# Duy1230/Map-Reduced-Approach-for-Vietnamese-Long-Document-Summarization

Measured on AMD Instinct MI355X. Metric: map-phase chunks/sec (2k-tok chunk, 256-tok summary) at 1/2/4/8 MI355X, higher is better.
Workload: dtype f16

## Files before the change

include/mapsum.h:

```cpp
#ifndef MAPSUM_H
#define MAPSUM_H

#include <stddef.h>
#include <stdint.h>

#ifdef __cplusplus
extern "C" {
#endif

#define MS_ABI_VERSION 3

#define MS_OK 0
#define MS_EIO -5
#define MS_ENOMEM -12
#define MS_EBUSY -16
#define MS_EINVAL -22
#define MS_ENOSPC -28

#define MS_FINISH_EOS 1
#define MS_FINISH_LENGTH 2
#define MS_FINISH_ERROR 3

#define MS_FLAG_IGNORE_EOS 1u

// ... 44 lines not shown
  int64_t finished;
  double prefill_ms, decode_ms;
  double kernel_ms[8];
  int64_t kernel_launches[8];
  int64_t decode_kv_tokens;
  int64_t graphs_built;
  int64_t persist_fallbacks;
  int64_t persist_steps;
} ms_stats;

typedef struct ms_engine ms_engine;

int ms_create(const ms_config* cfg, ms_engine** out);
int ms_destroy(ms_engine* e);
const char* ms_last_error(const ms_engine* e);

int ms_load_weight(ms_engine* e, int32_t tensor, int32_t layer, const uint16_t* host_f16,
                   int64_t n_elems);
int ms_init_synthetic(ms_engine* e, uint64_t seed, float std, float norm_jitter);

#define MS_GGML_Q4_K 12
#define MS_GGML_Q6_K 14
int ms_load_weight_q(ms_engine* e, int32_t tensor, int32_t layer, int32_t ggml_type,
                     const void* host_blocks, int64_t n_bytes);
int ms_init_synthetic_q(ms_engine* e, uint64_t seed, float scale, float norm_jitter);

int ms_weight_regions(const ms_engine* e, void** ptrs, int64_t* bytes, int32_t cap);
int ms_quant_manifest(const ms_engine* e, int32_t* triples, int32_t cap);
int ms_declare_weight_q(ms_engine* e, int32_t tensor, int32_t layer, int32_t ggml_type);

int ms_submit(ms_engine* e, const int32_t* ids, int32_t n, int32_t num_predict,
              uint32_t flags, uint64_t tag);
#define MS_SAMPLE_MAX_TOPK 256
#define MS_SAMPLE_MAX_WINDOW 256
typedef struct ms_sampling {
  float temperature;
  int32_t top_k;
  float top_p;
  float min_p;
  float repeat_penalty;
  int32_t repeat_last_n;
  uint64_t seed;
} ms_sampling;
int ms_submit_sampled(ms_engine* e, const int32_t* ids, int32_t n, int32_t num_predict,
                      uint32_t flags, uint64_t tag, const ms_sampling* sp);
int ms_set_eos_ids(ms_engine* e, const int32_t* ids, int32_t n);
int ms_step(ms_engine* e);
int ms_poll(ms_engine* e, ms_result* out, int32_t cap);
int ms_pending(const ms_engine* e);
int ms_get_stats(const ms_engine* e, ms_stats* out);
int ms_reset_stats(ms_engine* e);
int ms_set_profiling(ms_engine* e, uint32_t class_mask);
int ms_trace_push(const char* name);
int ms_trace_pop(void);
int ms_synchronize(ms_engine* e);
int ms_set_persist(ms_engine* e, int32_t on);
#define MS_DBG_KPOOL 0
#define MS_DBG_VPOOL 1
#define MS_DBG_DECODE_LOGITS 2
#define MS_DBG_DECODE_X 3
#define MS_DBG_PREFILL_LOGITS 4
int ms_debug_read(ms_engine* e, int32_t which, int64_t offset, void* host, int64_t bytes);
int ms_debug_pk_stamps(uint64_t* out, int32_t n);
int ms_debug_a2_stamps(uint64_t* out, int32_t n);

int ms_forward(ms_engine* e, const int32_t* ids, int32_t n, int32_t n_layers_run,
               float* hidden_out, float* logits_out);
int ms_forward_packed(ms_engine* e, const int32_t* ids, const int32_t* lens, int32_t n_seqs,
                      int32_t n_layers_run, float* hidden_out, float* logits_out);
int ms_submit_forced(ms_engine* e, const int32_t* ids, int32_t n, const int32_t* forced,
                     int32_t n_forced, int32_t num_predict, uint32_t flags, uint64_t tag);

#define MS_EPI_STORE_F16 0
#define MS_EPI_ADD_F32 1
#define MS_EPI_SWIGLU 2
#define MS_EPI_STORE_F32 3
#define MS_EPI_ARGMAX 5
int ms_op_gemm(const void* A, const void* W, void* out, int32_t M, int32_t N, int32_t K,
               int32_t ldo, int32_t epilogue, void* stream);
int ms_op_gemm_resid(const void* A, const void* W, float* x, void* xg_out, const void* gamma, float* ssq_out,
                     int32_t M, int32_t N, int32_t K, void* stream);
int ms_gemm_resid_tiles(int32_t M, int32_t N);
int ms_set_gemm_variant(int32_t variant);
int ms_set_qgemv_gs(int32_t on);
int ms_set_attn_tuning(int32_t combine_grp, int32_t order);
int ms_set_dgemm_kh(int32_t kh);
int ms_set_dgemm_wn(int32_t wn);
int64_t ms_op_gemv_workspace(int32_t M, int32_t N, int32_t K);
int ms_op_gemv(const void* X, const void* W, void* out, int32_t M, int32_t N, int32_t K,
               int32_t ldo, int32_t epilogue, void* workspace, void* stream);
int ms_op_gemv_tuned(const void* X, const void* W, void* out, int32_t M, int32_t N, int32_t K,
                     int32_t ldo, int32_t epilogue, void* workspace, int32_t waves, void* stream);
int ms_op_gemv_strided(const void* X, const void* W, void* out, int32_t M, int32_t N, int32_t K,
                       int32_t ldk, int32_t ldo, int32_t epilogue, void* stream);
int ms_op_gemv_resid(const void* X, const void* W, float* x, void* xg_out, const void* gamma,
                     float* ssq_out, int32_t M, int32_t N, int32_t K, int32_t rt, void* stream);
int ms_op_set_row_scale(const float* ssq, int32_t tiles, int32_t hidden, float eps);
int ms_op_dgemm(const void* X, const void* W, void* out, int32_t M, int32_t N, int32_t K, int32_t S,
                int32_t ldo, int32_t epilogue, void* stream);
int ms_op_gemv_split(const void* X, const void* W, float* slabs, int32_t M, int32_t N, int32_t K,
                     int32_t S, int32_t waves, void* stream);
int ms_op_residual_rmsnorm(float* x, const float* slabs, int32_t S, const void* w, void* y, float* ssq,
                           int32_t rows, int32_t hidden, void* stream);
int ms_op_dequant(int32_t ggml_type, const void* blocks, int64_t n_blocks, float* out, void* stream);
int ms_op_quant_rows(int32_t ggml_type, const void* blocks, int32_t rows, int32_t K, void* f16_out,
                     void* packed_out, void* stream);
int ms_op_qgemv(const void* X, int32_t ggml_type, const void* packed_rows, void* out, int32_t M,
                int32_t N, int32_t K, int32_t ldo, int32_t epilogue, void* stream);
int ms_op_qgemv_split(const void* X, int32_t ggml_type, const void* packed_rows, float* slabs,
                      int32_t M, int32_t N, int32_t K, int32_t S, void* stream);
int ms_op_qdgemm(const void* X, int32_t ggml_type, const void* packed_rows, void* out, int32_t M,
                 int32_t N, int32_t K, int32_t S, int32_t ldo, int32_t epilogue, void* stream);
int ms_op_rmsnorm(const void* x, const void* w, void* y, float* ssq, int32_t rows, int32_t hidden,
                  const int32_t* row_idx, void* stream);
int ms_op_argmax(const void* logits, int32_t rows, int32_t n, int32_t* ids, void* stream);
int ms_op_argmax_partials(const void* partials, int32_t rows, int32_t tiles, int32_t* ids, void* stream);
int ms_op_sample(const float* logits, int32_t rows, int32_t n, int64_t ldl, const ms_sampling* params,
                 const int32_t* win, const int32_t* win_len, const int32_t* steps, int32_t* ids,
                 int32_t* cand_ids, float* cand_p, int32_t* cand_n, void* stream);

#ifdef __cplusplus
}
#endif
#endif
```

map-reduced-approach-for-vietnamese-long-document-summarization_amd/csrc/engine.cpp:

```cpp
#include <hip/hip_runtime.h>

#include <algorithm>
#include <cmath>
#include <cstddef>
#include <cstdio>
#include <cstdlib>
#include <cstring>
#include <deque>
#include <array>
#include <functional>
#include <map>
#include <tuple>
#include <memory>
#include <stdexcept>
#include <string>
#include <vector>

#if MS_HAVE_ROCTX
#include <rocprofiler-sdk-roctx/roctx.h>
#else
static inline int roctxRangePushA(const char*) { return 0; }
static inline int roctxRangePop() { return 0; }
#endif

// ... 1803 lines not shown
    } catch (...) {
      if (lg) (void)hipFree(lg);
      for (Seq& s : seqs) release(E, s);
      throw;
    }
    if (lg) (void)hipFree(lg);
    for (Seq& s : seqs) release(E, s);
    E.ev_pending.clear();
    E.ev_used = 0;
    return MS_OK;
  });
}

int ms_forward(ms_engine* e, const int32_t* ids, int32_t n, int32_t n_layers_run, float* hidden_out,
               float* logits_out) {
  return ms_forward_packed(e, ids, &n, 1, n_layers_run, hidden_out, logits_out);
}

static int op_guard(const std::function<void()>& fn) {
  try {
    fn();
    hipError_t err = hipGetLastError();
    if (err != hipSuccess) {
      g_last_error = std::string("kernel launch failed: ") + hipGetErrorString(err);
      return MS_EIO;
    }
    return MS_OK;
  } catch (const MsError& x) {
    g_last_error = x.what();
    return x.code;
  }
}

static thread_local RowScale g_op_rs{};

int ms_op_set_row_scale(const float* ssq, int32_t tiles, int32_t hidden, float eps) {
  if (ssq && (tiles < 1 || hidden < 1)) return MS_EINVAL;
  g_op_rs = ssq ? make_row_scale(ssq, tiles, hidden, eps) : RowScale{};
  return MS_OK;
}

static int op_rs_tiles() { return g_op_rs.ssq ? g_op_rs.tiles : 0; }

static const GemvArgs* op_gemv_args(GemvArgs& ga) {
  ga = GemvArgs{};
  ga.rs = g_op_rs;
  return g_op_rs.ssq ? &ga : nullptr;
}

int ms_op_gemm(const void* A, const void* W, void* out, int32_t M, int32_t N, int32_t K, int32_t ldo,
               int32_t epi, void* stream) {
  return op_guard([&] {
    REQUIRE(A && W && out && M >= 1 && N >= 16 && K >= 64 && K % 64 == 0, MS_EINVAL, "bad gemm shape");
    REQUIRE(((epi >= 0 && epi <= 3) || epi == MS_EPI_ARGMAX) && (epi != MS_EPI_SWIGLU || N % 32 == 0), MS_EINVAL,
            "bad epilogue");
    REQUIRE(epi != MS_EPI_ADD_F32 || (N % 4 == 0 && ldo % 4 == 0), MS_EINVAL,
            "residual gemm: N and ldo multiples of 4 (16-B x rows)");
    REQUIRE(epi != MS_EPI_ARGMAX || (N % 16 == 0 && ldo >= N / 16), MS_EINVAL, "gemm argmax: N % 16, ldo >= N / 16");
    REQUIRE(((uintptr_t)out & ((epi == MS_EPI_ADD_F32 || epi == MS_EPI_STORE_F32) ? 15 : 7)) == 0, MS_EINVAL,
            "gemm: out must be 16-B (fp32) / 8-B (fp16) aligned");
    REQUIRE(!g_op_rs.ssq || gemm_rs_tiles_ok(M, N, g_op_rs.tiles), MS_EINVAL,
            "gemm row scale: at most 24 tiles of statistics (kGemmRsTiles, both GEMM tiles)");
    launch_gemm((const f16_t*)A, (const f16_t*)W, out, M, N, K, ldo, epi == MS_EPI_ARGMAX ? MS_GEMV_EPI_ARGMAX : epi,
                (hipStream_t)stream, &g_op_rs);
  });
}

int ms_op_gemm_resid(const void* A, const void* W, float* x, void* xg_out, const void* gamma, float* ssq_out,
                     int32_t M, int32_t N, int32_t K, void* stream) {
  return op_guard([&] {
    REQUIRE(A && W && x && xg_out && gamma && ssq_out && M >= 1 && N >= 16 && K >= 64 && K % 64 == 0, MS_EINVAL,
            "bad gemm_resid operands (K % 64 == 0)");
    REQUIRE(gemm_resid_tiles(M, N) <= kGemmRsTiles, MS_EINVAL, "gemm_resid: N over 24 column tiles");
    REQUIRE(N % 4 == 0 && ((uintptr_t)x & 15) == 0 && ((uintptr_t)xg_out & 7) == 0, MS_EINVAL,
            "gemm_resid: N a multiple of 4, x 16-B and xg 8-B aligned (vector rows)");
    GemmResid gr{(const f16_t*)gamma, (f16_t*)xg_out, ssq_out};
    launch_gemm((const f16_t*)A, (const f16_t*)W, x, M, N, K, N, MS_EPI_ADD_F32, (hipStream_t)stream, nullptr, &gr);
  });
}

int ms_gemm_resid_tiles(int32_t M, int32_t N) { return gemm_resid_tiles(M, N); }

int ms_set_gemm_variant(int32_t v) {
  if (v < 0 || v > 4) return MS_EINVAL;
  set_gemm_variant(v);
  return MS_OK;
}

int ms_set_attn_tuning(int32_t combine_grp, int32_t order) {
  if (combine_grp < 0 || combine_grp > 1 || (order != 0 && order != 3)) return MS_EINVAL;
  set_attn_tuning(combine_grp, order);
  return MS_OK;
}

int ms_set_dgemm_kh(int32_t kh) {
  if (kh != 1 && kh != 2) return MS_EINVAL;
  set_dgemm_kh(kh);
  return MS_OK;
}

int ms_set_dgemm_wn(int32_t wn) {
  if (wn != 4 && wn != 8) return MS_EINVAL;
  set_dgemm_wn(wn);
  return MS_OK;
}

int ms_set_qgemv_gs(int32_t on) {
  if (on < 0 || on > 1) return MS_EINVAL;
  set_qgemv_gs(on != 0);
  return MS_OK;
}

int64_t ms_op_gemv_workspace(int32_t M, int32_t N, int32_t K) {
  if (M < 1 || M > 64 || N < 16 || K < 64 || K % 64) return MS_EINVAL;
  return (int64_t)gemv_workspace_bytes(M, N, K);
}

int ms_op_gemv(const void* X, const void* W, void* out, int32_t M, int32_t N, int32_t K, int32_t ldo,
               int32_t epi, void* ws, void* stream) {
  return ms_op_gemv_tuned(X, W, out, M, N, K, ldo, epi, ws, 0, stream);
}

int ms_op_gemv_tuned(const void* X, const void* W, void* out, int32_t M, int32_t N, int32_t K,
                     int32_t ldo, int32_t epi, void* ws, int32_t waves, void* stream) {
  return op_guard([&] {
    REQUIRE(X && W && out && ws && N >= 16 && N % 16 == 0, MS_EINVAL, "bad gemv operands");
    REQUIRE(((epi >= 0 && epi <= 3) || epi == MS_EPI_ARGMAX) && (epi != MS_EPI_SWIGLU || N % 32 == 0),
            MS_EINVAL, "bad epilogue");
    REQUIRE(gemv_supported(M, N, K, epi, op_rs_tiles()), MS_EINVAL,
            "gemv shape unsupported (M<=64, K%64==0, K/64 split into <=16 waves of <=8 steps; "
            "row-scale statistics within kRsStage and LDS)");
    GemvArgs ga;
    launch_gemv_ex((const f16_t*)X, (const f16_t*)W, out, M, N, K, ldo, epi, op_gemv_args(ga), waves,
                   (hipStream_t)stream);
  });
}

int ms_op_gemv_strided(const void* X, const void* W, void* out, int32_t M, int32_t N, int32_t K,
                       int32_t ldk, int32_t ldo, int32_t epi, void* stream) {
  return op_guard([&] {
    REQUIRE(X && W && out && N >= 16 && N % 16 == 0 && ldk >= K && ldk % 8 == 0, MS_EINVAL,
            "bad strided gemv operands");
    REQUIRE(epi >= 0 && epi <= 3 && epi != MS_EPI_SWIGLU, MS_EINVAL, "bad epilogue");
    REQUIRE(gemv_supported(M, N, K, epi), MS_EINVAL, "gemv shape unsupported");
    launch_gemv_strided((const f16_t*)X, (const f16_t*)W, out, M, N, K, ldk, ldo, epi, (hipStream_t)stream);
  });
}

int ms_op_gemv_resid(const void* X, const void* W, float* x, void* xg_out, const void* gamma,
                     float* ssq_out, int32_t M, int32_t N, int32_t K, int32_t rt, void* stream) {
  return op_guard([&] {
    REQUIRE(X && W && x && xg_out && gamma && ssq_out && rt >= 1 && rt <= 16 && N % rt == 0, MS_EINVAL,
            "bad gemv_resid operands");
    REQUIRE(gemv_supported(M, N, K, MS_GEMV_EPI_RESID_SSQ), MS_EINVAL, "gemv_resid shape unsupported");
    GemvArgs ga{};
    ga.rt = rt;
    ga.ssq_out = ssq_out;
    ga.gamma = (const f16_t*)gamma;
    ga.xg_out = (f16_t*)xg_out;
    launch_gemv_ex((const f16_t*)X, (const f16_t*)W, x, M, N, K, N, MS_GEMV_EPI_RESID_SSQ, &ga, 0,
                   (hipStream_t)stream);
  });
}

int ms_op_dgemm(const void* X, const void* W, void* out, int32_t M, int32_t N, int32_t K, int32_t S,
                int32_t ldo, int32_t epi, void* stream) {
  return op_guard([&] {
    REQUIRE(X && W && out, MS_EINVAL, "bad dgemm operands");
// ... 164 lines not shown
```

map-reduced-approach-for-vietnamese-long-document-summarization_amd/csrc/k_gemm.hip:

```cpp
#include "kernels.h"

namespace ms {

constexpr int GBM = 128, GBN = 128, GBK = 64;

__device__ __forceinline__ int xcd_remap(int b, int nwg) {
  const int q = nwg / 8, r = nwg % 8, x = b % 8;
  return (x < r ? x * (q + 1) : r * (q + 1) + (x - r) * q) + b / 8;
}

__device__ __forceinline__ float silu_mul(float g, float u) {
  return g * __builtin_amdgcn_rcpf(1.0f + __expf(-g)) * u;
}

template <int BM, int NW>
__device__ __forceinline__ void gemm_rs_dma(const RowScale& rs, int M, int m0, float* rinv_s, float* stage) {
  if (!rs.ssq) return;
  const int lane = threadIdx.x & 63, wave = threadIdx.x >> 6;
  if (rs.tiles == 1) {
    if (wave < BM / 64)
      __builtin_amdgcn_global_load_lds((const void*)(rs.ssq + min(m0 + wave * 64 + lane, M - 1)),
                                       (LDS_AS void*)(rinv_s + wave * 64), 4, 0, 0);
    return;
  }
// ... 578 lines not shown
      mf1(1, 4 * g + 3);
      __builtin_amdgcn_sched_barrier(0);
    }
    __builtin_amdgcn_s_setprio(0);
  }
  asm volatile("s_nop 7\n\ts_nop 7\n\ts_nop 7\n\ts_nop 7" ::: "memory");

  if constexpr (EPI == 1) {
    const bool fuse = gr.xg != nullptr;
    float* red = (float*)smem;
    if (fuse) __syncthreads();
#pragma unroll
    for (int mi = 0; mi < 8; ++mi) {
      const int row = m0 + wr * 128 + mi * 16 + fr;
      float ss[2] = {0.f, 0.f};
#pragma unroll
      for (int ni = 0; ni < 8; ++ni) {
        const int col = n0 + wc * 128 + ni * 16 + 4 * fg;
        if (row < M && col < N)
          gemm_resid_x4(gr, (float*)out, (size_t)row * ldo + col, acc[mi][ni], g8[ni], fuse, ss[ni >> 2]);
      }
      if (fuse)
#pragma unroll
        for (int h = 0; h < 2; ++h) red[((wr * 128 + mi * 16 + fr) * 2 + wc) * 8 + h * 4 + fg] = ss[h];
    }
    if (fuse) gemm_resid_ssq_t<TBM, 2>(red, M, N, m0, n0, gr);
    return;
  }
  gemm_rs_fold<TBM, kGemmRsTiles>(rs, rinv_s, rs_stage);
  {
    float rv[8];
#pragma unroll
    for (int mi = 0; mi < 8; ++mi) rv[mi] = 1.f;
    if (rs.ssq) {
#pragma unroll
      for (int mi = 0; mi < 8; ++mi) rv[mi] = rs_rinv(rinv_s[wr * 128 + mi * 16 + fr], rs);
    }
    const bool vec = (ldo & 3) == 0;
#pragma unroll
    for (int mi = 0; mi < 8; ++mi) {
      const int row = m0 + wr * 128 + mi * 16 + fr;
      if (row >= M) continue;
      if constexpr (EPI == 2) {
#pragma unroll
        for (int ni = 0; ni < 8; ni += 2) {
          const int col = n0 + wc * 128 + ni * 16;
          if (col >= N) continue;
          const int f = (col >> 5) * 16 + 4 * fg;
          float hv[4];
#pragma unroll
          for (int j = 0; j < 4; ++j) hv[j] = silu_mul(acc[mi][ni][j] * rv[mi], acc[mi][ni + 1][j] * rv[mi]);
          f16_t* o = (f16_t*)out + (size_t)row * ldo + f;
          if (vec) {
            *(uint2*)o = uint2{pack2h(hv[0], hv[1]), pack2h(hv[2], hv[3])};
          } else {
#pragma unroll
            for (int j = 0; j < 4; ++j) o[j] = f2h(hv[j]);
          }
        }
      } else {
#pragma unroll
        for (int ni = 0; ni < 8; ++ni) {
          const int col = n0 + wc * 128 + ni * 16 + 4 * fg;
          if (col >= N) continue;
          const size_t o = (size_t)row * ldo + col;
          const f32x4 v = acc[mi][ni] * rv[mi];
          if (vec && col + 3 < N) {
            if constexpr (EPI == 0) *(uint2*)((f16_t*)out + o) = uint2{pack2h(v[0], v[1]), pack2h(v[2], v[3])};
            else *(f32x4*)((float*)out + o) = v;
          } else {
#pragma unroll
            for (int j = 0; j < 4; ++j)
              if (col + j < N) {
                if constexpr (EPI == 0) ((f16_t*)out)[o + j] = f2h(v[j]);
                else ((float*)out)[o + j] = v[j];
              }
          }
        }
      }
    }
  }
}

static int g_gemm_variant = [] { const char* e = getenv("MS_GEMM_VARIANT"); return e ? atoi(e) : 4; }();

void set_gemm_variant(int v) { g_gemm_variant = v; }

static bool gemm_big(int M, int N) {
  return g_gemm_variant == 2 || g_gemm_variant == 3 ||
         ((g_gemm_variant == 0 || g_gemm_variant == 4) && M >= 1024 && N >= 1024);
}
static bool gemm_4wave(int epi) { return g_gemm_variant == 3 || (g_gemm_variant == 4 && epi != 1); }

int gemm_resid_tiles(int M, int N) {
  (void)M;
  return (N + kGemmStatCols - 1) / kGemmStatCols;
}

void launch_gemm(const f16_t* A, const f16_t* W, void* out, int M, int N, int K, int ldo, int epi,
                 hipStream_t s, const RowScale* rs_in, const GemmResid* gr_in) {
  if (M <= 0) return;
  if (epi == MS_GEMV_EPI_ARGMAX) {
    const int grid = ((M + GBM - 1) / GBM) * ((N + GBN - 1) / GBN);
    MS_LAUNCH(gemm_kernel<MS_GEMV_EPI_ARGMAX>, dim3(grid), dim3(256), 0, s, A, W, out, M, N, K, ldo, RowScale{},
              GemmResid{});
    return;
  }
  const bool big = gemm_big(M, N);
  RowScale rs{};
  if (rs_in && rs_in->ssq && epi != 1) {
    if (rs_in->tiles < 1 || rs_in->tiles > kGemmRsTiles) return;
    rs = *rs_in;
  }
  GemmResid gr{};
  if (gr_in && epi == 1) gr = *gr_in;
#define GL(KERN, EPI_, BLK) MS_LAUNCH(KERN<EPI_>, dim3(grid), dim3(BLK), 0, s, A, W, out, M, N, K, ldo, rs, gr)
  if (big && gemm_4wave(epi) && K % TBK == 0) {
    const int grid = ((M + TBM - 1) / TBM) * ((N + TBN - 1) / TBN);
    switch (epi) {
      case 0: GL(gemm4w_kernel, 0, 256); break;
      case 1: GL(gemm4w_kernel, 1, 256); break;
      case 2: GL(gemm4w_kernel, 2, 256); break;
      default: GL(gemm4w_kernel, 3, 256); break;
    }
    return;
  }
  if (big) {
    const int grid = ((M + TBM - 1) / TBM) * ((N + TBN - 1) / TBN);
    switch (epi) {
      case 0: GL(gemm256_kernel, 0, 512); break;
      case 1: GL(gemm256_kernel, 1, 512); break;
      case 2: GL(gemm256_kernel, 2, 512); break;
      default: GL(gemm256_kernel, 3, 512); break;
    }
    return;
  }
  const int grid = ((M + GBM - 1) / GBM) * ((N + GBN - 1) / GBN);
  switch (epi) {
    case 0: GL(gemm_kernel, 0, 256); break;
    case 1: GL(gemm_kernel, 1, 256); break;
    case 2: GL(gemm_kernel, 2, 256); break;
    default: GL(gemm_kernel, 3, 256); break;
  }
#undef GL
}

bool gemm_rs_tiles_ok(int M, int N, int tiles) {
  (void)M;
  (void)N;
  return tiles >= 1 && tiles <= kGemmRsTiles;
}

}
```

map-reduced-approach-for-vietnamese-long-document-summarization_amd/csrc/kernels.h:

```cpp
#pragma once
#include "common.h"

namespace ms {

struct KVView {
  f16_t* k;
  f16_t* v;
  const int32_t* block_table;
  int32_t max_pages;
  int32_t n_kv_heads;
  int32_t slot_major;
};

constexpr int kPrefillQRows = 128;
struct PrefillAttnArgs {
  const int32_t* seq_qstart;
  const int32_t* seq_qlen;
  const int32_t* seq_kvlen;
  const int32_t* seq_slot;
  const int32_t* qblk;
  int32_t n_qblk;
  const float* cos_tab;
  const float* sin_tab;
};
// ... 1 lines not shown
struct DecodeAttnArgs {
  const int32_t* seq_len;
  const int32_t* seq_slot;
  int32_t B;
  int32_t max_len;
  int32_t ppw;
};

struct RowScale {
  const float* ssq;
  int tiles, H;
  float eps;
  float inv_h;
};
inline RowScale make_row_scale(const float* ssq, int tiles, int H, float eps) {
  return RowScale{ssq, tiles, H, eps, 1.0f / (float)H};
}
constexpr float kXgScale = 0.0625f, kXgUnscale = 16.0f;
__device__ __forceinline__ float rs_rinv(float sum, const RowScale& rs) {
  return __builtin_amdgcn_rsqf(__fmaf_rn(sum, rs.inv_h, rs.eps)) * kXgUnscale;
}

void launch_embed(const int32_t* ids, int T, const f16_t* emb, int H, float* x, hipStream_t s,
                  const f16_t* gamma = nullptr, f16_t* xg = nullptr, float* ssq = nullptr);
void launch_decode_advance(int32_t* args, const int32_t* ids_out, int32_t* ring, int B, int V,
                           hipStream_t s);
void launch_decode_tail(const void* partials, int tiles, int32_t* args, int32_t* ids_out, int32_t* ring, int B,
                        int V, const f16_t* emb, int H, float* x, const f16_t* gamma, f16_t* xg, float* ssq,
                        hipStream_t s);
void launch_rmsnorm(const float* x, const f16_t* w, f16_t* y, float* ssq, int rows, int H,
                    const int32_t* row_idx, hipStream_t s);
void launch_rope_kv(f16_t* qkv, int T, int Hq, int Hk, const int32_t* tok_pos,
                    const int32_t* tok_slot, const float* cos_tab, const float* sin_tab,
                    KVView kv, hipStream_t s, bool rope_q = true);
void launch_argmax(const float* logits, int rows, int n, int32_t* out, hipStream_t s);

constexpr int kSampleMaxTopK = 256, kSampleMaxWindow = 256;
constexpr int kSampleMaxN = 131072;
struct SampleParams {
  float temperature;
  int32_t top_k;
  float top_p, min_p, repeat_penalty;
  int32_t repeat_last_n;
  uint64_t seed;
};
struct SampleSlot {
  SampleParams p;
  int32_t wcount;
  int32_t step;
  int32_t ring[kSampleMaxWindow];
};
struct SampleArgs {
  const float* logits;
  int64_t ldl;
  int n;
  const SampleParams* params;
  const int32_t* win;
  const int32_t* win_len;
  const int32_t* steps;
  SampleSlot* slots;
  const int32_t* row_slot;
  int32_t* ids_out;
  int32_t* cand_ids;
  float* cand_p;
  int32_t* cand_n;
};
void launch_sample_rows(const SampleArgs& a, int rows, hipStream_t s);
void launch_sample_tail(const float* logits, SampleSlot* slots, int32_t* args, int32_t* ids_out, int32_t* ring,
                        int B, int V, const f16_t* emb, int H, float* x, const f16_t* gamma, f16_t* xg, float* ssq,
                        hipStream_t s);

struct GemmResid {
  const f16_t* gamma;
  f16_t* xg;
  float* ssq;
};
constexpr int kGemmRsTiles = 24;
constexpr int kGemmStatCols = 128;
int gemm_resid_tiles(int M, int N);
bool gemm_rs_tiles_ok(int M, int N, int tiles);
void launch_gemm(const f16_t* A, const f16_t* W, void* out, int M, int N, int K, int ldo,
                 int epi, hipStream_t s, const RowScale* rs = nullptr, const GemmResid* gr = nullptr);
void set_gemm_variant(int v);
void set_qgemv_gs(bool on);
void set_attn_tuning(int combine_grp, int order);
void set_dgemm_kh(int kh);
void set_dgemm_wn(int wn);
enum {
  MS_GEMV_EPI_STORE_F16 = 0,
  MS_GEMV_EPI_ADD_F32 = 1,
  MS_GEMV_EPI_SWIGLU = 2,
  MS_GEMV_EPI_STORE_F32 = 3,
  MS_GEMV_EPI_ROPE_KV = 4,
  MS_GEMV_EPI_ARGMAX = 5,
  MS_GEMV_EPI_RESID_SSQ = 6
};
struct GemvArgs {
  const int32_t* tok_pos;
  const int32_t* tok_slot;
  const float* cos_tab;
  const float* sin_tab;
  KVView kv;
  int Hq, Hk;
  int rt;
  float* ssq_out;
  const f16_t* gamma;
  f16_t* xg_out;
  RowScale rs;
  int slab_rows;
};
bool gemv_split_supported(int M, int N, int K, int S, int rs_tiles = 0);
bool gemv_rs_supported(int M, int tiles);
void launch_gemv_split(const f16_t* X, const f16_t* W, float* slabs, int M, int N, int K, int S,
                       int force_waves, hipStream_t s, const GemvArgs* ga = nullptr);
void launch_gemv_strided(const f16_t* X, const f16_t* W, void* out, int M, int N, int K, int ldk,
                         int ldo, int epi, hipStream_t s);
void launch_argmax_partials(const void* partials, int rows, int tiles, int32_t* out, hipStream_t s);

bool residual_rmsnorm_supported(int S, int H);
void launch_residual_rmsnorm(float* x, const float* slabs, int S, const f16_t* w, f16_t* y,
                             float* ssq, int rows, int H, hipStream_t s);
size_t gemv_workspace_bytes(int M, int N, int K);
bool gemv_supported(int M, int N, int K, int epi, int rs_tiles = 0);
void launch_gemv(const f16_t* X, const f16_t* W, void* out, int M, int N, int K, int ldo,
                 int epi, void* ws, hipStream_t s);
void launch_gemv_ex(const f16_t* X, const f16_t* W, void* out, int M, int N, int K, int ldo,
                    int epi, const GemvArgs* ga, int force_waves, hipStream_t s);

bool dgemm_supported(int M, int N, int K, int S, int epi, int kh = 0, int wn = 0);
void launch_dgemm(const f16_t* X, const f16_t* W, void* out, int M, int N, int K, int S, int ldo, int epi,
                  hipStream_t s, const RowScale* rs = nullptr, int kh = 0, int wn = 0);
int dgemm_kh_setting();

enum { MS_QT_Q4_K = 12, MS_QT_Q6_K = 14 };
constexpr int kQ4KBytes = 144, kQ6KBytes = 210, kQ6KPacked = 224;
struct QMat {
  int n;
  const uint8_t* base0; int row0_0, type0, row_bytes0;
  const uint8_t* base1; int row0_1, type1, row_bytes1;
  const uint8_t* base2; int row0_2, type2, row_bytes2;
};
bool qdgemm_supported(int M, int N, int K, int S, int epi, const QMat& q);
void launch_qdgemm(const f16_t* X, const QMat& q, void* out, int M, int N, int K, int S, int ldo, int epi,
                   hipStream_t s, const RowScale* rs = nullptr);
bool qdgemm_f16_supported(int M, int N, int K, int S, int epi);
void launch_qdgemm_f16(const f16_t* X, const f16_t* W, void* out, int M, int N, int K, int S, int ldo, int epi,
                       hipStream_t s, const RowScale* rs = nullptr);

inline uint64_t smix_host(uint64_t z) {
  z += 0x9E3779B97F4A7C15ull;
  z = (z ^ (z >> 30)) * 0xBF58476D1CE4E5B9ull;
  z = (z ^ (z >> 27)) * 0x94D049BB133111EBull;
  return z ^ (z >> 31);
}
inline int qblock_bytes(int type, bool packed) {
  return type == MS_QT_Q4_K ? kQ4KBytes : (packed ? kQ6KPacked : kQ6KBytes);
}
void launch_dequant_f32(int type, const uint8_t* blocks, int64_t n_blocks, float* out, hipStream_t s);
void launch_quant_rows(int type, const uint8_t* blocks, int rows, int K, f16_t* dst_f16,
                       int map_mul, int map_add, uint8_t* dst_q, int q_row_base, hipStream_t s);
void launch_synth_qblocks(int type, uint8_t* blocks, int64_t n_blocks, uint64_t seed, float scale,
                          hipStream_t s);
bool qgemv_supported(int M, int N, int K, int epi, int rs_tiles = 0);
bool qgemv_split_supported(int M, int N, int K, int S, int rs_tiles = 0);
void launch_qgemv_split(const f16_t* X, const QMat& q, float* slabs, int M, int N, int K, int S,
                        hipStream_t s, const GemvArgs* ga = nullptr);
// ... 90 lines not shown
```

map-reduced-approach-for-vietnamese-long-document-summarization_amd/mapsum/_lib.py:

```python
from __future__ import annotations

import ctypes as C
import os

_HERE = os.path.dirname(os.path.abspath(__file__))
LIB_PATH = os.environ.get("MAPSUM_LIB") or os.path.join(_HERE, "libmapsum.so")

MS_ABI_VERSION = 3
MS_OK, MS_EIO, MS_ENOMEM, MS_EBUSY, MS_EINVAL, MS_ENOSPC = 0, -5, -12, -16, -22, -28
MS_FINISH_EOS, MS_FINISH_LENGTH, MS_FINISH_ERROR = 1, 2, 3
MS_FLAG_IGNORE_EOS = 1
(MS_T_EMBED, MS_T_ATTN_NORM, MS_T_WQ, MS_T_WK, MS_T_WV, MS_T_WO, MS_T_FFN_NORM, MS_T_WGATE,
 MS_T_WUP, MS_T_WDOWN, MS_T_FINAL_NORM, MS_T_LM_HEAD) = range(12)
MS_EPI_STORE_F16, MS_EPI_ADD_F32, MS_EPI_SWIGLU, MS_EPI_STORE_F32 = range(4)
MS_EPI_ARGMAX = 5
GEMM_DEFAULT = 4
MS_GGML_Q4_K, MS_GGML_Q6_K = 12, 14
K_GEMM, K_ATTN_PREFILL, K_GEMV, K_ATTN_DECODE, K_LMHEAD, K_MISC, K_PERSIST = range(7)
MS_DBG_KPOOL, MS_DBG_VPOOL, MS_DBG_DECODE_LOGITS, MS_DBG_DECODE_X, MS_DBG_PREFILL_LOGITS = range(5)
MS_SAMPLE_MAX_TOPK, MS_SAMPLE_MAX_WINDOW = 256, 256

EXPORTED = (
    "ms_create", "ms_destroy", "ms_last_error", "ms_load_weight", "ms_init_synthetic",
    "ms_load_weight_q", "ms_init_synthetic_q", "ms_op_dequant", "ms_op_quant_rows", "ms_op_qgemv", "ms_op_qgemv_split", "ms_op_qdgemm",
    "ms_submit", "ms_step", "ms_poll", "ms_pending", "ms_get_stats", "ms_reset_stats",
    "ms_set_profiling", "ms_synchronize", "ms_forward", "ms_op_gemm", "ms_op_gemv_workspace",
    "ms_op_gemv", "ms_op_gemv_tuned", "ms_op_gemv_split", "ms_op_dgemm", "ms_op_residual_rmsnorm", "ms_op_rmsnorm",
    "ms_op_argmax", "ms_op_argmax_partials", "ms_set_gemm_variant", "ms_set_qgemv_gs", "ms_set_attn_tuning", "ms_set_dgemm_kh", "ms_set_dgemm_wn",
    "ms_weight_regions", "ms_quant_manifest", "ms_declare_weight_q",
    "ms_forward_packed", "ms_submit_forced", "ms_set_eos_ids", "ms_op_gemv_strided",
    "ms_op_gemv_resid", "ms_op_set_row_scale", "ms_op_gemm_resid", "ms_gemm_resid_tiles",
    "ms_trace_push", "ms_trace_pop", "ms_debug_a2_stamps", "ms_set_persist", "ms_debug_read", "ms_debug_pk_stamps",
    "ms_submit_sampled", "ms_op_sample",
)


class MsConfig(C.Structure):
    _fields_ = [("abi_version", C.c_int32),
                ("n_layers", C.c_int32), ("hidden", C.c_int32), ("n_heads", C.c_int32),
                ("n_kv_heads", C.c_int32), ("head_dim", C.c_int32), ("ffn", C.c_int32),
                ("vocab", C.c_int32),
                ("rope_theta", C.c_float), ("rope_factor", C.c_float),
                ("rope_low_freq_factor", C.c_float), ("rope_high_freq_factor", C.c_float),
                ("rope_orig_ctx", C.c_int32), ("norm_eps", C.c_float), ("tie_embeddings", C.c_int32),
                ("device", C.c_int32), ("max_batch", C.c_int32), ("max_ctx", C.c_int32),
                ("max_prefill_tokens", C.c_int32), ("n_pages", C.c_int32), ("n_eos", C.c_int32),
                ("eos_ids", C.c_int32 * 8)]


class MsSampling(C.Structure):
    _fields_ = [("temperature", C.c_float), ("top_k", C.c_int32), ("top_p", C.c_float),
                ("min_p", C.c_float), ("repeat_penalty", C.c_float), ("repeat_last_n", C.c_int32),
                ("seed", C.c_uint64)]


class MsResult(C.Structure):
    _fields_ = [("tag", C.c_uint64), ("ids", C.POINTER(C.c_int32)), ("n_ids", C.c_int32),
                ("finish_reason", C.c_int32), ("n_prompt", C.c_int32), ("_pad", C.c_int32)]


class MsStats(C.Structure):
    _fields_ = [("prefill_tokens", C.c_int64), ("decode_tokens", C.c_int64),
                ("prefill_passes", C.c_int64), ("decode_steps", C.c_int64), ("finished", C.c_int64),
                ("prefill_ms", C.c_double), ("decode_ms", C.c_double),
                ("kernel_ms", C.c_double * 8), ("kernel_launches", C.c_int64 * 8),
                ("decode_kv_tokens", C.c_int64), ("graphs_built", C.c_int64),
                ("persist_fallbacks", C.c_int64), ("persist_steps", C.c_int64)]


_lib = None


def load() -> C.CDLL:
    global _lib
    if _lib is not None:
        return _lib
    if not os.path.exists(LIB_PATH):
        raise RuntimeError(f"libmapsum.so not found at {LIB_PATH}; build it with "
                           f"`make -C csrc` or `python -c 'import __graft_entry__ as g; g.build()'`")
    _lib = load_at(LIB_PATH, bool(os.environ.get("MAPSUM_LIB")))
    return _lib


def load_at(path: str, ab: bool = True) -> C.CDLL:
    lib = C.CDLL(path)
    vp, i32, i64, u32, u64 = C.c_void_p, C.c_int32, C.c_int64, C.c_uint32, C.c_uint64
    pi32 = C.POINTER(C.c_int32)
    sig = {
        "ms_create": (i32, [C.POINTER(MsConfig), C.POINTER(vp)]),
        "ms_destroy": (i32, [vp]),
        "ms_last_error": (C.c_char_p, [vp]),
        "ms_load_weight": (i32, [vp, i32, i32, vp, i64]),
        "ms_init_synthetic": (i32, [vp, u64, C.c_float, C.c_float]),
        "ms_load_weight_q": (i32, [vp, i32, i32, i32, vp, i64]),
        "ms_init_synthetic_q": (i32, [vp, u64, C.c_float, C.c_float]),
        "ms_op_dequant": (i32, [i32, vp, i64, vp, vp]),
        "ms_op_quant_rows": (i32, [i32, vp, i32, i32, vp, vp, vp]),
        "ms_op_qgemv": (i32, [vp, i32, vp, vp, i32, i32, i32, i32, i32, vp]),
        "ms_op_qgemv_split": (i32, [vp, i32, vp, vp, i32, i32, i32, i32, vp]),
        "ms_op_qdgemm": (i32, [vp, i32, vp, vp, i32, i32, i32, i32, i32, i32, vp]),
        "ms_submit": (i32, [vp, pi32, i32, i32, u32, u64]),
        "ms_submit_sampled": (i32, [vp, pi32, i32, i32, u32, u64, C.POINTER(MsSampling)]),
        "ms_op_sample": (i32, [vp, i32, i32, i64, vp, vp, vp, vp, vp, vp, vp, vp, vp]),
        "ms_step": (i32, [vp]),
        "ms_poll": (i32, [vp, C.POINTER(MsResult), i32]),
        "ms_pending": (i32, [vp]),
        "ms_get_stats": (i32, [vp, C.POINTER(MsStats)]),
        "ms_reset_stats": (i32, [vp]),
        "ms_set_profiling": (i32, [vp, u32]),
        "ms_synchronize": (i32, [vp]),
        "ms_forward": (i32, [vp, pi32, i32, i32, vp, vp]),
        "ms_forward_packed": (i32, [vp, pi32, pi32, i32, i32, vp, vp]),
        "ms_set_eos_ids": (i32, [vp, pi32, i32]),
        "ms_op_gemv_strided": (i32, [vp, vp, vp, i32, i32, i32, i32, i32, i32, vp]),
        "ms_op_gemv_resid": (i32, [vp, vp, vp, vp, vp, vp, i32, i32, i32, i32, vp]),
        "ms_op_set_row_scale": (i32, [vp, i32, i32, C.c_float]),
        "ms_op_gemm_resid": (i32, [vp, vp, vp, vp, vp, vp, i32, i32, i32, vp]),
        "ms_gemm_resid_tiles": (i32, [i32, i32]),
        "ms_submit_forced": (i32, [vp, pi32, i32, pi32, i32, i32, u32, u64]),
        "ms_op_gemm": (i32, [vp, vp, vp, i32, i32, i32, i32, i32, vp]),
        "ms_op_gemv_workspace": (i64, [i32, i32, i32]),
        "ms_op_gemv": (i32, [vp, vp, vp, i32, i32, i32, i32, i32, vp, vp]),
        "ms_op_gemv_tuned": (i32, [vp, vp, vp, i32, i32, i32, i32, i32, vp, i32, vp]),
        "ms_op_gemv_split": (i32, [vp, vp, vp, i32, i32, i32, i32, i32, vp]),
        "ms_op_dgemm": (i32, [vp, vp, vp, i32, i32, i32, i32, i32, i32, vp]),
        "ms_op_residual_rmsnorm": (i32, [vp, vp, i32, vp, vp, vp, i32, i32, vp]),
        "ms_op_rmsnorm": (i32, [vp, vp, vp, vp, i32, i32, vp, vp]),
        "ms_set_gemm_variant": (i32, [i32]),
        "ms_set_qgemv_gs": (i32, [i32]),
        "ms_set_attn_tuning": (i32, [i32, i32]),
        "ms_set_dgemm_kh": (i32, [i32]),
        "ms_set_dgemm_wn": (i32, [i32]),
        "ms_op_argmax": (i32, [vp, i32, i32, vp, vp]),
        "ms_op_argmax_partials": (i32, [vp, i32, i32, vp, vp]),
        "ms_weight_regions": (i32, [vp, C.POINTER(vp), C.POINTER(i64), i32]),
        "ms_quant_manifest": (i32, [vp, pi32, i32]),
        "ms_declare_weight_q": (i32, [vp, i32, i32, i32]),
        "ms_trace_push": (i32, [C.c_char_p]),
        "ms_trace_pop": (i32, []),
        "ms_set_persist": (i32, [vp, i32]),
        "ms_debug_read": (i32, [vp, i32, i64, vp, i64]),
        "ms_debug_pk_stamps": (i32, [vp, i32]),
        "ms_debug_a2_stamps": (i32, [vp, i32]),
    }
    for name, (res, args) in sig.items():
        if ab and not hasattr(lib, name):
            continue
        fn = getattr(lib, name)
        fn.restype = res
        fn.argtypes = args
    return lib


def check(rc: int, handle=None, what: str = "") -> int:
    if rc < 0:
        msg = load().ms_last_error(handle)
        raise RuntimeError(f"libmapsum {what} failed ({rc}): {msg.decode() if msg else ''}")
    return rc


class trace:

    def __init__(self, name: str):
        self.name = name.encode()
        self.lib = None

    def __enter__(self):
        try:
            lib = load()
            if hasattr(lib, "ms_trace_push"):
                lib.ms_trace_push(self.name)
                self.lib = lib
        except (OSError, RuntimeError):
            self.lib = None
        return self

    def __exit__(self, *exc):
        if self.lib is not None:
            self.lib.ms_trace_pop()
        return False
```

Baseline: 12.86.

## Add persistent tile-looping GEMM for residual-add epilogue, default on

Adds a persistent 256x256 GEMM kernel for the residual-add (epi==1) path. Each block, launched once per CU, loops over output tiles and issues the next tile's prologue DMA and residual loads while it is still running the current tile's epilogue and row-sum-of-squares reduction. The aim is to hide per-tile startup and epilogue latency and to cut the tail from uneven tile waves. The default variant becomes 5, so prefill residual GEMMs take this path. The risk is lower occupancy, since each block needs 128KB+ of LDS, and heavier scheduling complexity.

```diff
diff --git a/include/mapsum.h b/include/mapsum.h
--- a/include/mapsum.h
+++ b/include/mapsum.h
@@ -150,6 +150,7 @@
                      int32_t M, int32_t N, int32_t K, void* stream);
 int ms_gemm_resid_tiles(int32_t M, int32_t N);
 int ms_set_gemm_variant(int32_t variant);
+int ms_set_gemm_loop_blocks(int32_t n);
 int ms_set_qgemv_gs(int32_t on);
 int ms_set_attn_tuning(int32_t combine_grp, int32_t order);
 int ms_set_dgemm_kh(int32_t kh);
diff --git a/map-reduced-approach-for-vietnamese-long-document-summarization_amd/csrc/engine.cpp b/map-reduced-approach-for-vietnamese-long-document-summarization_amd/csrc/engine.cpp
--- a/map-reduced-approach-for-vietnamese-long-document-summarization_amd/csrc/engine.cpp
+++ b/map-reduced-approach-for-vietnamese-long-document-summarization_amd/csrc/engine.cpp
@@ -1909,8 +1909,14 @@
 int ms_gemm_resid_tiles(int32_t M, int32_t N) { return gemm_resid_tiles(M, N); }
 
 int ms_set_gemm_variant(int32_t v) {
-  if (v < 0 || v > 4) return MS_EINVAL;
+  if (v < 0 || v > 6) return MS_EINVAL;
   set_gemm_variant(v);
+  return MS_OK;
+}
+
+int ms_set_gemm_loop_blocks(int32_t n) {
+  if (n < 0) return MS_EINVAL;
+  set_gemm_loop_blocks(n);
   return MS_OK;
 }
 
diff --git a/map-reduced-approach-for-vietnamese-long-document-summarization_amd/csrc/k_gemm.hip b/map-reduced-approach-for-vietnamese-long-document-summarization_amd/csrc/k_gemm.hip
--- a/map-reduced-approach-for-vietnamese-long-document-summarization_amd/csrc/k_gemm.hip
+++ b/map-reduced-approach-for-vietnamese-long-document-summarization_amd/csrc/k_gemm.hip
@@ -684,15 +684,204 @@
   }
 }
 
-static int g_gemm_variant = [] { const char* e = getenv("MS_GEMM_VARIANT"); return e ? atoi(e) : 4; }();
+__global__ __launch_bounds__(512, 1) void gemm256_loop_kernel(const f16_t* __restrict__ A,
+                                                             const f16_t* __restrict__ W,
+                                                             float* __restrict__ x, int M, int N, int K,
+                                                             int ldo, GemmResid gr) {
+  __shared__ __attribute__((aligned(16))) char smem[2 * 65536 + TBM * 2 * 8 * 4];
+  float* red = (float*)(smem + 2 * 65536);
+  const int tid = threadIdx.x, lane = tid & 63;
+  const int wave = __builtin_amdgcn_readfirstlane(tid >> 6);
+  const int tiles_m = (M + TBM - 1) / TBM, tiles_n = (N + TBN - 1) / TBN;
+  const int ntiles = tiles_m * tiles_n;
+  const int wr = wave >> 2, wc = wave & 3;
+  const int fr = lane & 15, fg = lane >> 4;
+  const int sw = fr >> 1;
+
+  int m0 = 0, n0 = 0;
+  uint32_t src_off[4][2];
+  auto unit_row = [&](int u, int i, int r) {
+    const int lr = (2 * wave + i) * 8 + r;
+    if (u == 0) return lr < 64 ? lr : lr + 64;
+    if (u == 1) return lr < 64 ? lr + 64 : lr + 128;
+    return (lr >> 5) * 64 + (lr & 31) + (u == 3 ? 32 : 0);
+  };
+  auto setup = [&](int tile) {
+    const int pid = xcd_remap(tile, ntiles);
+    constexpr int GM = 8;
+    const int grp = pid / (GM * tiles_n);
+    const int first_m = grp * GM;
+    const int gsz = min(tiles_m - first_m, GM);
+    const int in_grp = pid % (GM * tiles_n);
+    m0 = (first_m + in_grp % gsz) * TBM;
+    n0 = (in_grp / gsz) * TBN;
+#pragma unroll
+    for (int u = 0; u < 4; ++u)
+#pragma unroll
+      for (int i = 0; i < 2; ++i) {
+        const int tr = unit_row(u, i, lane >> 3);
+        const int grow = u < 2 ? min(m0 + tr, M - 1) : min(n0 + tr, N - 1);
+        src_off[u][i] = (uint32_t)grow * (uint32_t)K + (uint32_t)(((lane & 7) ^ swz2(tr)) * 8);
+      }
+  };
+  const uint32_t lds0 = __builtin_amdgcn_readfirstlane((uint32_t)(uintptr_t)(LDS_AS char*)smem);
+  auto stage = [&](int buf, int u, int k0) {
+    const f16_t* base = u < 2 ? A : W;
+#pragma unroll
+    for (int i = 0; i < 2; ++i) {
+      const f16_t* src = base + src_off[u][i] + k0;
+      const uint32_t dst = lds0 + buf * 65536 + (u < 2 ? 0 : 32768) + unit_row(u, i, 0) * 128;
+      asm volatile("s_nop 0\n\tglobal_load_lds_dwordx4 %1, off" ::"{m0}"(dst), "v"(src) : "memory");
+    }
+  };
+
+  f32x4 acc[8][4];
+  uint2 g4[4];
+  f16x8 af[4][2], bfr[2][2];
+  auto read_a = [&](int buf, int qa) {
+    const char* img = smem + buf * 65536;
+#pragma unroll
+    for (int m = 0; m < 4; ++m)
+#pragma unroll
+      for (int s2 = 0; s2 < 2; ++s2) {
+        const int row = wr * 128 + qa * 64 + m * 16 + fr;
+        af[m][s2] = *(const f16x8*)(img + row * 128 + (((4 * s2 + fg) ^ sw) << 4));
+      }
+  };
+  auto read_b = [&](int buf, int qb) {
+    const char* img = smem + buf * 65536 + 32768;
+#pragma unroll
+    for (int n = 0; n < 2; ++n)
+#pragma unroll
+      for (int s2 = 0; s2 < 2; ++s2) {
+        const int row = wc * 64 + qb * 32 + n * 16 + fr;
+        bfr[n][s2] = *(const f16x8*)(img + row * 128 + (((4 * s2 + fg) ^ sw) << 4));
+      }
+  };
+  auto mma = [&](int qa, int qb) {
+    __builtin_amdgcn_s_barrier();
+    asm volatile("s_waitcnt lgkmcnt(0)" ::: "memory");
+    __builtin_amdgcn_sched_barrier(0);
+    __builtin_amdgcn_s_setprio(1);
+#pragma unroll
+    for (int m = 0; m < 4; ++m)
+#pragma unroll
+      for (int n = 0; n < 2; ++n)
+#pragma unroll
+        for (int s2 = 0; s2 < 2; ++s2)
+          acc[qa * 4 + m][qb * 2 + n] = mfma16(bfr[n][s2], af[m][s2], acc[qa * 4 + m][qb * 2 + n]);
+    __builtin_amdgcn_s_setprio(0);
+    __builtin_amdgcn_s_barrier();
+  };
+  const f16_t* gp = gr.xg ? gr.gamma : (const f16_t*)A;
+  auto load_x = [&]() {
+#pragma unroll
+    for (int mi = 0; mi < 8; ++mi)
+#pragma unroll
+      for (int ni = 0; ni < 4; ++ni) {
+        const int row = min(m0 + wr * 128 + mi * 16 + fr, M - 1);
+        const int col = min(n0 + wc * 64 + ni * 16 + 4 * fg, N - 4);
+        acc[mi][ni] = *(const f32x4*)(x + (size_t)row * ldo + col);
+      }
+#pragma unroll
+    for (int ni = 0; ni < 4; ++ni) g4[ni] = *(const uint2*)(gp + min(n0 + wc * 64 + ni * 16 + 4 * fg, N - 4));
+  };
+  const int nk = K / TBK;
+  auto prologue_dma = [&]() {
+    stage(0, 0, 0);
+    stage(0, 3, 0);
+    stage(0, 1, 0);
+    stage(0, 2, 0);
+    if (nk > 1) {
+      stage(1, 0, TBK);
+      stage(1, 3, TBK);
+    }
+  };
+
+  int tile = blockIdx.x;
+  setup(tile);
+  prologue_dma();
+  load_x();
+  const bool fuse = gr.xg != nullptr;
+  for (;;) {
+    __builtin_amdgcn_s_waitcnt((0x7 << 4) | (0xF << 8));
+    __builtin_amdgcn_s_barrier();
+    if (wr == 1) __builtin_amdgcn_s_barrier();
+
+    for (int t = 0; t < nk; ++t) {
+      const int buf = t & 1, nb = buf ^ 1;
+      const bool has1 = t + 1 < nk, has2 = t + 2 < nk;
+      read_b(buf, 0);
+      __builtin_amdgcn_sched_barrier(0);
+      read_a(buf, 0);
+      if (has1) stage(nb, 1, (t + 1) * TBK);
+      mma(0, 0);
+      read_b(buf, 1);
+      if (has1) stage(nb, 2, (t + 1) * TBK);
+      mma(0, 1);
+      read_a(buf, 1);
+      if (has2) stage(buf, 0, (t + 2) * TBK);
+      mma(1, 1);
+      read_b(buf, 0);
+      if (has2) {
+        stage(buf, 3, (t + 2) * TBK);
+        asm volatile("s_waitcnt vmcnt(4)" ::: "memory");
+      } else {
+        asm volatile("s_waitcnt vmcnt(0)" ::: "memory");
+      }
+      mma(1, 0);
+    }
+    if (wr == 0) __builtin_amdgcn_s_barrier();
+
+    const int em0 = m0, en0 = n0;
+    const int next = tile + (int)gridDim.x;
+    const bool more = next < ntiles;
+    if (more) {
+      setup(next);
+      prologue_dma();
+    }
+#pragma unroll
+    for (int mi = 0; mi < 8; ++mi) {
+      const int row = em0 + wr * 128 + mi * 16 + fr;
+      float ss = 0.f;
+#pragma unroll
+      for (int ni = 0; ni < 4; ++ni) {
+        const int col = en0 + wc * 64 + ni * 16 + 4 * fg;
+        if (row < M && col < N) gemm_resid_x4(gr, x, (size_t)row * ldo + col, acc[mi][ni], g4[ni], fuse, ss);
+      }
+      if (fuse) red[((wr * 128 + mi * 16 + fr) * 2 + (wc >> 1)) * 8 + (wc & 1) * 4 + fg] = ss;
+    }
+    if (more) load_x();
+    if (fuse) gemm_resid_ssq_t<TBM, 2>(red, M, N, em0, en0, gr);
+    if (!more) break;
+    tile = next;
+  }
+}
+
+static int g_gemm_variant = [] { const char* e = getenv("MS_GEMM_VARIANT"); return e ? atoi(e) : 5; }();
+static int g_gemm_loop_blocks = 0;
 
 void set_gemm_variant(int v) { g_gemm_variant = v; }
+void set_gemm_loop_blocks(int n) { g_gemm_loop_blocks = n; }
 
 static bool gemm_big(int M, int N) {
-  return g_gemm_variant == 2 || g_gemm_variant == 3 ||
-         ((g_gemm_variant == 0 || g_gemm_variant == 4) && M >= 1024 && N >= 1024);
-}
-static bool gemm_4wave(int epi) { return g_gemm_variant == 3 || (g_gemm_variant == 4 && epi != 1); }
+  return g_gemm_variant == 2 || g_gemm_variant == 3 || g_gemm_variant == 6 ||
+         ((g_gemm_variant == 0 || g_gemm_variant == 4 || g_gemm_variant == 5) && M >= 1024 && N >= 1024);
+}
+static bool gemm_4wave(int epi) {
+  return g_gemm_variant == 3 || ((g_gemm_variant == 4 || g_gemm_variant == 5) && epi != 1);
+}
+static bool gemm_loop(int epi) { return (g_gemm_variant == 5 || g_gemm_variant == 6) && epi == 1; }
+static int gemm_n_cu() {
+  static const int n = [] {
+    int dev = 0, cu = 0;
+    if (hipGetDevice(&dev) != hipSuccess ||
+        hipDeviceGetAttribute(&cu, hipDeviceAttributeMultiprocessorCount, dev) != hipSuccess || cu < 1)
+      cu = 256;
+    return cu;
+  }();
+  return n;
+}
 
 int gemm_resid_tiles(int M, int N) {
   (void)M;
@@ -717,6 +906,13 @@
   GemmResid gr{};
   if (gr_in && epi == 1) gr = *gr_in;
 #define GL(KERN, EPI_, BLK) MS_LAUNCH(KERN<EPI_>, dim3(grid), dim3(BLK), 0, s, A, W, out, M, N, K, ldo, rs, gr)
+  if (big && gemm_loop(epi) && K % TBK == 0) {
+    const int tiles = ((M + TBM - 1) / TBM) * ((N + TBN - 1) / TBN);
+    const int cap = g_gemm_loop_blocks > 0 ? g_gemm_loop_blocks : gemm_n_cu();
+    const int grid = tiles < cap ? tiles : cap;
+    MS_LAUNCH(gemm256_loop_kernel, dim3(grid), dim3(512), 0, s, A, W, (float*)out, M, N, K, ldo, gr);
+    return;
+  }
   if (big && gemm_4wave(epi) && K % TBK == 0) {
     const int grid = ((M + TBM - 1) / TBM) * ((N + TBN - 1) / TBN);
     switch (epi) {
diff --git a/map-reduced-approach-for-vietnamese-long-document-summarization_amd/csrc/kernels.h b/map-reduced-approach-for-vietnamese-long-document-summarization_amd/csrc/kernels.h
--- a/map-reduced-approach-for-vietnamese-long-document-summarization_amd/csrc/kernels.h
+++ b/map-reduced-approach-for-vietnamese-long-document-summarization_amd/csrc/kernels.h
@@ -107,6 +107,7 @@
 void launch_gemm(const f16_t* A, const f16_t* W, void* out, int M, int N, int K, int ldo,
                  int epi, hipStream_t s, const RowScale* rs = nullptr, const GemmResid* gr = nullptr);
 void set_gemm_variant(int v);
+void set_gemm_loop_blocks(int n);
 void set_qgemv_gs(bool on);
 void set_attn_tuning(int combine_grp, int order);
 void set_dgemm_kh(int kh);
diff --git a/map-reduced-approach-for-vietnamese-long-document-summarization_amd/mapsum/_lib.py b/map-reduced-approach-for-vietnamese-long-document-summarization_amd/mapsum/_lib.py
--- a/map-reduced-approach-for-vietnamese-long-document-summarization_amd/mapsum/_lib.py
+++ b/map-reduced-approach-for-vietnamese-long-document-summarization_amd/mapsum/_lib.py
@@ -14,7 +14,7 @@
  MS_T_WUP, MS_T_WDOWN, MS_T_FINAL_NORM, MS_T_LM_HEAD) = range(12)
 MS_EPI_STORE_F16, MS_EPI_ADD_F32, MS_EPI_SWIGLU, MS_EPI_STORE_F32 = range(4)
 MS_EPI_ARGMAX = 5
-GEMM_DEFAULT = 4
+GEMM_DEFAULT = 5
 MS_GGML_Q4_K, MS_GGML_Q6_K = 12, 14
 K_GEMM, K_ATTN_PREFILL, K_GEMV, K_ATTN_DECODE, K_LMHEAD, K_MISC, K_PERSIST = range(7)
 MS_DBG_KPOOL, MS_DBG_VPOOL, MS_DBG_DECODE_LOGITS, MS_DBG_DECODE_X, MS_DBG_PREFILL_LOGITS = range(5)
@@ -31,7 +31,7 @@
     "ms_forward_packed", "ms_submit_forced", "ms_set_eos_ids", "ms_op_gemv_strided",
     "ms_op_gemv_resid", "ms_op_set_row_scale", "ms_op_gemm_resid", "ms_gemm_resid_tiles",
     "ms_trace_push", "ms_trace_pop", "ms_debug_a2_stamps", "ms_set_persist", "ms_debug_read", "ms_debug_pk_stamps",
-    "ms_submit_sampled", "ms_op_sample",
+    "ms_submit_sampled", "ms_op_sample", "ms_set_gemm_loop_blocks",
 )
 
 
@@ -127,6 +127,7 @@
         "ms_op_residual_rmsnorm": (i32, [vp, vp, i32, vp, vp, vp, i32, i32, vp]),
         "ms_op_rmsnorm": (i32, [vp, vp, vp, vp, i32, i32, vp, vp]),
         "ms_set_gemm_variant": (i32, [i32]),
+        "ms_set_gemm_loop_blocks": (i32, [i32]),
         "ms_set_qgemv_gs": (i32, [i32]),
         "ms_set_attn_tuning": (i32, [i32, i32]),
         "ms_set_dgemm_kh": (i32, [i32]),
```

Result: no change. 12.86 (-0.0%).
